# Sbte/RAILS

Measured on AMD Instinct MI355X. Metric: RAILS iterations/sec (+ A*V SpMM HBM GB/s in roofline), m=1M rows/GPU, k=128, fp64, higher is better.
Workload: dtype f64

## Files before the change

### include/rails_hip.h

```cpp
#ifndef RAILS_HIP_H
#define RAILS_HIP_H

#include <stddef.h>
#include <stdint.h>

#ifdef __cplusplus
extern "C" {
#endif

#define RAILS_OK 0
#define RAILS_EINVAL -1
#define RAILS_EHIP -2
#define RAILS_ENOMEM -3
#define RAILS_ELAPACK -4
#define RAILS_ECOMM -5
#define RAILS_ENODEV -6

typedef struct rails_ctx rails_ctx;
typedef struct rails_csr rails_csr;
typedef struct rails_panel rails_panel;

const char *rails_last_error(void);
const char *rails_version(void);


int rails_ctx_create(int device, void *stream, rails_ctx **out);
int rails_ctx_destroy(rails_ctx *ctx);
int rails_ctx_sync(rails_ctx *ctx);
void *rails_ctx_stream(rails_ctx *ctx);
int rails_ctx_stats(rails_ctx *ctx, char *buf, int cap);
int rails_ctx_set_meter(rails_ctx *ctx, int on);

int rails_ctx_set_seed(rails_ctx *ctx, uint64_t seed, uint64_t first_stream);
int rails_ctx_rng_state(rails_ctx *ctx, uint64_t *seed, uint64_t *next_stream);

int rails_ctx_set_partition(rails_ctx *ctx, int rank, int nranks, int64_t row0, int64_t m_global);

typedef int (*rails_allreduce_fn)(void *user, double *dev_buf, size_t n, void *stream);
int rails_ctx_set_allreduce(rails_ctx *ctx, rails_allreduce_fn fn, void *user);

#define RAILS_RCCL_ID_BYTES 128
int rails_rccl_unique_id(void *id_out);
int rails_ctx_init_rccl(rails_ctx *ctx, const void *id, int nranks, int rank);
int rails_ctx_set_rccl(rails_ctx *ctx, void *nccl_comm);
int rails_ctx_rccl_size(const rails_ctx *ctx);

typedef int (*rails_halo_fn)(void *user, const double *send_buf, double *recv_buf, int ncols, void *stream);


int rails_csr_create(rails_ctx *ctx, int64_t m_local, int64_t n_cols_ext, const int64_t *rowptr,
                     const int32_t *col, const double *val, rails_csr **out);
typedef int (*rails_apply_fn)(void *user, int trans, const rails_panel *X, int xc0, int nc, rails_panel *Y, int yc0);
int rails_csr_create_callback(rails_ctx *ctx, int64_t m_local, rails_apply_fn fn, void *user, rails_csr **out);
int rails_csr_destroy(rails_csr *A);
int64_t rails_csr_rows(const rails_csr *A);
int64_t rails_csr_nnz(const rails_csr *A);

int rails_csr_set_halo(rails_csr *A, int64_t n_send, const int64_t *send_rows, int64_t n_ghost,
                       rails_halo_fn fn, void *user);

int rails_csr_set_halo_counts(rails_csr *A, int nranks, const int64_t *send_counts, const int64_t *recv_counts);

int rails_spmm(rails_ctx *ctx, rails_csr *A, int trans, const rails_panel *X, int xc0, int nc,
               rails_panel *Y, int yc0);

int rails_csr_set_variant(rails_csr *A, int variant);
int rails_csr_prepare(rails_ctx *ctx, rails_csr *A, int trans, int nc, int *kernel_ready);
int rails_csr_sweep_stats(rails_csr *A, int nc, double *out);
int rails_csr_tile_stats(rails_csr *A, double *out);
int rails_csr_create_rect(rails_ctx *ctx, int64_t n_rows, int64_t n_cols, const int64_t *rowptr, const int32_t *col, const double *val,
                          rails_csr **out);
const char *rails_csr_last_kernel(const rails_csr *A);

typedef struct rails_sptrsv rails_sptrsv;
int rails_sptrsv_create(rails_ctx *ctx, int64_t n, const int64_t *rowptr, const int32_t *col, const double *val, int lower, int unit_diag,
                        rails_sptrsv **out);
void rails_sptrsv_destroy(rails_sptrsv *T);
int64_t rails_sptrsv_levels(const rails_sptrsv *T);
int rails_sptrsv_solve(rails_ctx *ctx, const rails_sptrsv *T, rails_panel *X, int c0, int nc);
int rails_panel_permute_rows(rails_ctx *ctx, const rails_panel *X, int xc0, int nc, const int32_t *perm_dev, int scatter, rails_panel *Y, int yc0);
int rails_index_upload(rails_ctx *ctx, const int32_t *host, int64_t n, int32_t **out_dev);
void rails_index_free(rails_ctx *ctx, int32_t *dev);
// ... 41 lines not shown
typedef struct rails_sweep_plan rails_sweep_plan;
int rails_sweep_plan_create(int64_t m, int64_t ncols, const int64_t *rowptr, const int32_t *col, const double *val,
                            const int *params, rails_sweep_plan **out);
int rails_sweep_plan_destroy(rails_sweep_plan *plan);
int rails_sweep_plan_info(const rails_sweep_plan *plan, int64_t *iinfo, double *dinfo);
int rails_sweep_plan_array(const rails_sweep_plan *plan, int which, const void **ptr, int64_t *count);


int rails_panel_create(rails_ctx *ctx, int64_t m_local, int capacity, rails_panel **out);
int rails_panel_create_ld(rails_ctx *ctx, int64_t m_local, int capacity, int ld, rails_panel **out);
int rails_panel_destroy(rails_panel *P);
int64_t rails_panel_rows(const rails_panel *P);
int rails_panel_capacity(const rails_panel *P);
int rails_panel_ld(const rails_panel *P);
void *rails_panel_device_ptr(const rails_panel *P);
int rails_panel_reserve(rails_ctx *ctx, rails_panel *P, int capacity);

int rails_panel_upload(rails_ctx *ctx, rails_panel *P, int c0, int nc, const double *host, int64_t ldh);
int rails_panel_download(rails_ctx *ctx, const rails_panel *P, int c0, int nc, double *host, int64_t ldh);

int rails_panel_fill(rails_ctx *ctx, rails_panel *P, int c0, int nc, double value);
int rails_panel_scale(rails_ctx *ctx, rails_panel *P, int c0, int nc, double s);
int rails_panel_copy(rails_ctx *ctx, const rails_panel *X, int xc0, int nc, rails_panel *Y, int yc0);
int rails_panel_axpy(rails_ctx *ctx, double alpha, const rails_panel *X, int xc0, int nc, rails_panel *Y,
                     int yc0);
int rails_panel_random(rails_ctx *ctx, rails_panel *P, int c0, int nc);

int rails_gram(rails_ctx *ctx, const rails_panel *X, int xc0, int a, const rails_panel *Y, int yc0, int b,
               double *C_host, int ldc);

int rails_panel_gemm(rails_ctx *ctx, double alpha, const rails_panel *X, int xc0, int k, const double *C_host,
                     int ldc, int r, double beta, rails_panel *Y, int yc0);

int rails_ctx_enable_library_gemm(rails_ctx *ctx);
int rails_ctx_library_gemm_ready(const rails_ctx *ctx);

int rails_deferred_reserve(rails_ctx *ctx, int nslots, int64_t doubles_per_slot);
int rails_gram_deferred(rails_ctx *ctx, const rails_panel *X, int xc0, int a, const rails_panel *Y, int yc0, int b, int slot);
int rails_panel_gemm_deferred(rails_ctx *ctx, double alpha, const rails_panel *X, int xc0, int k, int slot, int ld, int r, double beta,
                              rails_panel *Y, int yc0);
int rails_chol_inverse_deferred(rails_ctx *ctx, int slot_in, int w, int slot_out);
int rails_update_gram_deferred(rails_ctx *ctx, double alpha, const rails_panel *X, int xc0, int k, const double *C_host, int ldc, int r,
                               rails_panel *Y, int yc0, int r2, int slot);
int rails_update_gram_deferred_out(rails_ctx *ctx, double alpha, const rails_panel *X, int xc0, int k, const double *C_host, int ldc, int r,
                                   const rails_panel *Y, int yc0, rails_panel *Yout, int oc0, int r2, int slot);
int rails_deferred_fetch(rails_ctx *ctx, int slot, int64_t n, double *host_out);

int rails_panel_gemm_wide(rails_ctx *ctx, double alpha, const rails_panel *X, int xc0, int k, const double *C_host, int ldc, int r,
                          double beta, rails_panel *Y, int yc0);

void rails_dense_set_tile_fit(int on);
int rails_dense_tile_fit(void);
int rails_dense_last_tiles(const rails_ctx *ctx, int *update_gram_nbw, int *gram_cols_ti, int *gemm_wide_tr);

int rails_orthogonalize(rails_ctx *ctx, rails_panel *V, int k_old, int w, int method, int *used);
int rails_orthogonalize_deflated(rails_ctx *ctx, rails_panel *V, int k_old, int w, const rails_panel *N, int nc0, int q, int method, int *used);

int rails_panel_colnorms2(rails_ctx *ctx, const rails_panel *X, int c0, int nc, double *out_host);

int rails_orthogonalize_range(rails_ctx *ctx, rails_panel *V, int k_old, int w, const rails_panel *N, int nc0, int q, double tol, int *kept,
                              int32_t *kept_idx);

int rails_resid_lanczos(rails_ctx *ctx, const rails_panel *AV, int avc0, const rails_panel *MV, int mvc0, int k,
                        const double *T_host, int ldt, const rails_panel *B, int bc0, int p, int L,
                        double *H_host, int ldh, int *steps);

int rails_resid_lanczos_sparse(rails_ctx *ctx, const rails_panel *AV, int avc0, const rails_panel *MV, int mvc0, int k, const double *T_host,
                               int ldt, const rails_sprhs *S, int L, double *H_host, int ldh, int *steps);

int rails_lanczos_start(rails_ctx *ctx, const rails_panel *AV, int avc0, const rails_panel *MV, int mvc0, int k,
                        const rails_panel *B, int bc0, int p, double *sums_host);

int rails_lanczos_vectors(rails_ctx *ctx, const double *S_host, int lds, int w, rails_panel *Out, int oc0);
int rails_lanczos_last_launch(rails_ctx *ctx, int *nch, int *unroll, int *nblocks);
int rails_lanczos_release(rails_ctx *ctx);

int rails_ctx_reserve_staging(rails_ctx *ctx, size_t bytes);
int rails_timer_start(rails_ctx *ctx);
int rails_timer_stop(rails_ctx *ctx, double *ms);


void rails_sb03md(char dico, char job, char fact, char trans, int n, double *A, int lda, double *X, int ldx,
                  double *scale, int *info);
void rails_sb03md_counts(long *smith, long *schur);
void rails_sb03md_adi_counts(long *extended, long *fresh);
void rails_sb03md_set_pause(int calls);
void rails_dsyev(char jobz, char uplo, int n, double *a, int lda, double *w, int *info);
void rails_dsteqr(char compz, int n, double *d, double *e, double *z, int ldz, double *work, int *info);
void rails_dgemm(char transa, char transb, int m, int n, int k, double alpha, const double *A, int lda, const double *B,
                 int ldb, double beta, double *C, int ldc);
void rails_dtrsm(char side, char uplo, char transa, char diag, int m, int n, double alpha, const double *A, int lda, double *B, int ldb);
void rails_dpotrf(char uplo, int n, double *a, int lda, int *info);
void rails_dpstrf(char uplo, int n, double *a, int lda, int *piv, int *rank, double tol, int *info);
void rails_range_basis(int m, int n, double *a, int lda, double tol, double *q, int ldq, int *rank, int *info);
int rails_host_lapack_init(const char *path);
const char *rails_host_lapack_path(void);

#ifdef __cplusplus
}
#endif
#endif
```

### rails_amd/_lib.py

```python
import ctypes as C
import os

_HERE = os.path.dirname(os.path.abspath(__file__))
LIB_PATH = os.path.join(_HERE, "lib", "librails_hip.so")

_dp = C.POINTER(C.c_double)
_ip = C.POINTER(C.c_int)
_i64p = C.POINTER(C.c_int64)
_i32p = C.POINTER(C.c_int32)
_vp = C.c_void_p

ALLREDUCE_FN = C.CFUNCTYPE(C.c_int, C.c_void_p, C.c_void_p, C.c_size_t, C.c_void_p)
HALO_FN = C.CFUNCTYPE(C.c_int, C.c_void_p, C.c_void_p, C.c_void_p, C.c_int, C.c_void_p)
APPLY_FN = C.CFUNCTYPE(C.c_int, C.c_void_p, C.c_int, C.c_void_p, C.c_int, C.c_int, C.c_void_p, C.c_int)

SIGNATURES = {
    "rails_last_error": (C.c_char_p, []),
    "rails_version": (C.c_char_p, []),
    "rails_ctx_create": (C.c_int, [C.c_int, _vp, C.POINTER(_vp)]),
    "rails_ctx_destroy": (C.c_int, [_vp]),
    "rails_ctx_sync": (C.c_int, [_vp]),
    "rails_ctx_stream": (_vp, [_vp]),
    "rails_ctx_set_meter": (C.c_int, [_vp, C.c_int]),
    "rails_ctx_enable_library_gemm": (C.c_int, [_vp]),
    "rails_ctx_library_gemm_ready": (C.c_int, [_vp]),
    "rails_deferred_reserve": (C.c_int, [_vp, C.c_int, C.c_int64]),
    "rails_gram_deferred": (C.c_int, [_vp, _vp, C.c_int, C.c_int, _vp, C.c_int, C.c_int, C.c_int]),
    "rails_update_gram_deferred": (C.c_int, [_vp, C.c_double, _vp, C.c_int, C.c_int, _dp, C.c_int, C.c_int, _vp, C.c_int, C.c_int, C.c_int]),
    "rails_update_gram_deferred_out": (C.c_int, [_vp, C.c_double, _vp, C.c_int, C.c_int, _dp, C.c_int, C.c_int, _vp, C.c_int, _vp, C.c_int, C.c_int, C.c_int]),
    "rails_panel_gemm_deferred": (C.c_int, [_vp, C.c_double, _vp, C.c_int, C.c_int, C.c_int, C.c_int, C.c_int, C.c_double, _vp, C.c_int]),
    "rails_chol_inverse_deferred": (C.c_int, [_vp, C.c_int, C.c_int, C.c_int]),
    "rails_deferred_fetch": (C.c_int, [_vp, C.c_int, C.c_int64, _dp]),
    "rails_ctx_stats": (C.c_int, [_vp, C.c_char_p, C.c_int]),
    "rails_ctx_set_seed": (C.c_int, [_vp, C.c_uint64, C.c_uint64]),
    "rails_ctx_rng_state": (C.c_int, [_vp, C.POINTER(C.c_uint64), C.POINTER(C.c_uint64)]),
    "rails_ctx_set_partition": (C.c_int, [_vp, C.c_int, C.c_int, C.c_int64, C.c_int64]),
    "rails_ctx_set_allreduce": (C.c_int, [_vp, ALLREDUCE_FN, _vp]),
    "rails_rccl_unique_id": (C.c_int, [_vp]),
    "rails_ctx_init_rccl": (C.c_int, [_vp, _vp, C.c_int, C.c_int]),
    "rails_ctx_set_rccl": (C.c_int, [_vp, _vp]),
    "rails_ctx_rccl_size": (C.c_int, [_vp]),
    "rails_csr_set_halo_counts": (C.c_int, [_vp, C.c_int, _i64p, _i64p]),
    "rails_csr_create": (C.c_int, [_vp, C.c_int64, C.c_int64, _i64p, _i32p, _dp, C.POINTER(_vp)]),
    "rails_csr_create_rect": (C.c_int, [_vp, C.c_int64, C.c_int64, _i64p, _i32p, _dp, C.POINTER(_vp)]),
    "rails_csr_create_callback": (C.c_int, [_vp, C.c_int64, APPLY_FN, _vp, C.POINTER(_vp)]),
    "rails_csr_destroy": (C.c_int, [_vp]),
    "rails_csr_rows": (C.c_int64, [_vp]),
    "rails_csr_nnz": (C.c_int64, [_vp]),
    "rails_csr_set_halo": (C.c_int, [_vp, C.c_int64, _i64p, C.c_int64, HALO_FN, _vp]),
    "rails_spmm": (C.c_int, [_vp, _vp, C.c_int, _vp, C.c_int, C.c_int, _vp, C.c_int]),
    "rails_csr_set_variant": (C.c_int, [_vp, C.c_int]),
    "rails_csr_sweep_stats": (C.c_int, [_vp, C.c_int, _dp]),
    "rails_csr_tile_stats": (C.c_int, [_vp, _dp]),
    "rails_csr_prepare": (C.c_int, [_vp, _vp, C.c_int, C.c_int, C.POINTER(C.c_int)]),
    "rails_csr_last_kernel": (C.c_char_p, [_vp]),
    "rails_sweep_plan_create": (C.c_int, [C.c_int64, C.c_int64, _i64p, _i32p, _dp, _ip, C.POINTER(_vp)]),
    "rails_sweep_plan_destroy": (C.c_int, [_vp]),
    "rails_sweep_plan_info": (C.c_int, [_vp, _i64p, _dp]),
    "rails_sweep_plan_array": (C.c_int, [_vp, C.c_int, C.POINTER(_vp), _i64p]),
    "rails_panel_create": (C.c_int, [_vp, C.c_int64, C.c_int, C.POINTER(_vp)]),
    "rails_panel_create_ld": (C.c_int, [_vp, C.c_int64, C.c_int, C.c_int, C.POINTER(_vp)]),
    "rails_panel_destroy": (C.c_int, [_vp]),
    "rails_panel_rows": (C.c_int64, [_vp]),
    "rails_panel_capacity": (C.c_int, [_vp]),
    "rails_panel_ld": (C.c_int, [_vp]),
    "rails_panel_device_ptr": (_vp, [_vp]),
    "rails_panel_reserve": (C.c_int, [_vp, _vp, C.c_int]),
    "rails_panel_upload": (C.c_int, [_vp, _vp, C.c_int, C.c_int, _dp, C.c_int64]),
    "rails_panel_download": (C.c_int, [_vp, _vp, C.c_int, C.c_int, _dp, C.c_int64]),
    "rails_panel_fill": (C.c_int, [_vp, _vp, C.c_int, C.c_int, C.c_double]),
    "rails_panel_scale": (C.c_int, [_vp, _vp, C.c_int, C.c_int, C.c_double]),
    "rails_panel_copy": (C.c_int, [_vp, _vp, C.c_int, C.c_int, _vp, C.c_int]),
    "rails_panel_axpy": (C.c_int, [_vp, C.c_double, _vp, C.c_int, C.c_int, _vp, C.c_int]),
    "rails_sptrsv_create": (C.c_int, [_vp, C.c_int64, _i64p, _i32p, _dp, C.c_int, C.c_int, C.POINTER(_vp)]),
    "rails_sptrsv_destroy": (None, [_vp]),
    "rails_sptrsv_levels": (C.c_int64, [_vp]),
    "rails_sptrsv_solve": (C.c_int, [_vp, _vp, _vp, C.c_int, C.c_int]),
    "rails_panel_permute_rows": (C.c_int, [_vp, _vp, C.c_int, C.c_int, _vp, C.c_int, _vp, C.c_int]),
    "rails_index_upload": (C.c_int, [_vp, _i32p, C.c_int64, C.POINTER(_vp)]),
    "rails_index_free": (None, [_vp, _vp]),
    "rails_lu_create": (C.c_int, [_vp, C.c_int64, _i64p, _i32p, _dp, _i64p, _i32p, _dp, _i32p, _i32p, _i32p, C.c_int64, C.POINTER(_vp)]),
    "rails_lu_destroy": (None, [_vp]),
    "rails_lu_solve": (C.c_int, [_vp, _vp, C.c_int, _vp, C.c_int, C.c_int, _vp, C.c_int]),
    "rails_lu_stats": (C.c_int, [_vp, _i64p, C.c_int]),
    "rails_csr_create_lu": (C.c_int, [_vp, _vp, C.POINTER(_vp)]),
    "rails_iter_create": (C.c_int, [_vp, _vp, C.c_int, _dp, C.POINTER(_vp)]),
    "rails_iter_set": (C.c_int, [_vp, C.c_char_p, C.c_double]),
    "rails_iter_solve": (C.c_int, [_vp, _vp, C.c_int, _vp, C.c_int, C.c_int, _vp, C.c_int]),
    "rails_iter_precondition": (C.c_int, [_vp, _vp, _vp, C.c_int, C.c_int, _vp, C.c_int]),
    "rails_iter_stats": (C.c_int, [_vp, _dp, C.c_int]),
    "rails_iter_columns": (C.c_int, [_vp, _i32p, _dp, _i32p, C.c_int]),
    "rails_csr_create_iter": (C.c_int, [_vp, _vp, C.POINTER(_vp)]),
    "rails_iter_destroy": (None, [_vp]),
    "rails_csr_transpose_host": (C.c_int, [C.c_int64, C.c_int64, _i64p, _i32p, _dp, _i64p, _i32p, _dp]),
    "rails_csr_gram_norm2_host": (C.c_int, [C.c_int64, C.c_int64, _i64p, _i32p, _dp, _i64p, _i32p, _dp, _dp]),
    "rails_sprhs_create": (C.c_int, [_vp, C.c_int64, C.c_int, _i64p, _i32p, _dp, C.POINTER(_vp)]),
    "rails_sprhs_destroy": (None, [_vp]),
    "rails_sprhs_rows": (C.c_int64, [_vp]),
    "rails_sprhs_cols": (C.c_int64, [_vp]),
    "rails_sprhs_nnz": (C.c_int64, [_vp]),
    "rails_sprhs_gram_norm2": (C.c_double, [_vp]),
    "rails_sprhs_apply": (C.c_int, [_vp, _vp, C.c_int, _vp, C.c_int, C.c_int, _vp, C.c_int]),
    "rails_csr_create_sprhs": (C.c_int, [_vp, _vp, C.POINTER(_vp)]),
    "rails_csr_cols": (C.c_int64, [_vp]),
    "rails_csr_sprhs": (_vp, [_vp]),
    "rails_resid_lanczos_sparse": (C.c_int, [_vp, _vp, C.c_int, _vp, C.c_int, C.c_int, _dp, C.c_int, _vp, C.c_int, _dp, C.c_int, _ip]),
    "rails_panel_random": (C.c_int, [_vp, _vp, C.c_int, C.c_int]),
    "rails_gram": (C.c_int, [_vp, _vp, C.c_int, C.c_int, _vp, C.c_int, C.c_int, _dp, C.c_int]),
    "rails_panel_gemm": (C.c_int, [_vp, C.c_double, _vp, C.c_int, C.c_int, _dp, C.c_int, C.c_int, C.c_double, _vp, C.c_int]),
    "rails_panel_gemm_wide": (C.c_int, [_vp, C.c_double, _vp, C.c_int, C.c_int, _dp, C.c_int, C.c_int, C.c_double, _vp, C.c_int]),
    "rails_dense_set_tile_fit": (None, [C.c_int]),
    "rails_dense_tile_fit": (C.c_int, []),
    "rails_dense_last_tiles": (C.c_int, [_vp, _ip, _ip, _ip]),
    "rails_orthogonalize": (C.c_int, [_vp, _vp, C.c_int, C.c_int, C.c_int, _ip]),
    "rails_orthogonalize_deflated": (C.c_int, [_vp, _vp, C.c_int, C.c_int, _vp, C.c_int, C.c_int, C.c_int, _ip]),
    "rails_panel_colnorms2": (C.c_int, [_vp, _vp, C.c_int, C.c_int, _dp]),
    "rails_orthogonalize_range": (C.c_int, [_vp, _vp, C.c_int, C.c_int, _vp, C.c_int, C.c_int, C.c_double, _ip, _i32p]),
    "rails_resid_lanczos": (C.c_int, [_vp, _vp, C.c_int, _vp, C.c_int, C.c_int, _dp, C.c_int, _vp, C.c_int, C.c_int, C.c_int,
                                      _dp, C.c_int, _ip]),
    "rails_lanczos_start": (C.c_int, [_vp, _vp, C.c_int, _vp, C.c_int, C.c_int, _vp, C.c_int, C.c_int, _dp]),
    "rails_lanczos_vectors": (C.c_int, [_vp, _dp, C.c_int, C.c_int, _vp, C.c_int]),
    "rails_lanczos_last_launch": (C.c_int, [_vp, _ip, _ip, _ip]),
    "rails_lanczos_release": (C.c_int, [_vp]),
    "rails_timer_start": (C.c_int, [_vp]),
    "rails_timer_stop": (C.c_int, [_vp, _dp]),
    "rails_sb03md": (None, [C.c_char, C.c_char, C.c_char, C.c_char, C.c_int, _dp, C.c_int, _dp, C.c_int, _dp, _ip]),
    "rails_dsyev": (None, [C.c_char, C.c_char, C.c_int, _dp, C.c_int, _dp, _ip]),
    "rails_dsteqr": (None, [C.c_char, C.c_int, _dp, _dp, _dp, C.c_int, _dp, _ip]),
    "rails_ctx_reserve_staging": (C.c_int, [_vp, C.c_size_t]),
    "rails_sb03md_set_pause": (None, [C.c_int]),
    "rails_sb03md_counts": (None, [C.POINTER(C.c_long), C.POINTER(C.c_long)]),
    "rails_sb03md_adi_counts": (None, [C.POINTER(C.c_long), C.POINTER(C.c_long)]),
    "rails_dtrsm": (None, [C.c_char, C.c_char, C.c_char, C.c_char, C.c_int, C.c_int, C.c_double, _dp, C.c_int, _dp, C.c_int]),
    "rails_dgemm": (None, [C.c_char, C.c_char, C.c_int, C.c_int, C.c_int, C.c_double, _dp, C.c_int, _dp, C.c_int, C.c_double, _dp, C.c_int]),
    "rails_dpotrf": (None, [C.c_char, C.c_int, _dp, C.c_int, _ip]),
    "rails_dpstrf": (None, [C.c_char, C.c_int, _dp, C.c_int, _ip, _ip, C.c_double, _ip]),
    "rails_range_basis": (None, [C.c_int, C.c_int, _dp, C.c_int, C.c_double, _dp, C.c_int, _ip, _ip]),
    "rails_host_lapack_init": (C.c_int, [C.c_char_p]),
    "rails_host_lapack_path": (C.c_char_p, []),
}

_lib = None


class RailsError(RuntimeError):
    pass


def load():
    global _lib
    if _lib is not None:
        return _lib
    if not os.path.exists(LIB_PATH):
        raise RailsError(
            "rails_amd: %s is missing -- build it with `python -c 'import __graft_entry__ as g; g.build()'` "
            "or `make -C rails_amd/csrc`; there is no CPU fallback" % LIB_PATH)
    lib = C.CDLL(LIB_PATH, mode=C.RTLD_GLOBAL)
    for name, (res, args) in SIGNATURES.items():
        fn = getattr(lib, name)
        fn.restype = res
        fn.argtypes = args
    try:
        from ._solver_sigs import bind as _bind_solver
        _bind_solver(lib)
    except ImportError:
        pass
# ... 12 lines not shown
```

### rails_amd/csrc/ctx.hip

```cpp
#include "rails_internal.h"

static thread_local char g_err[1024] = "";

void rails_set_error(const char *fmt, ...)
{
    va_list ap;
    va_start(ap, fmt);
    vsnprintf(g_err, sizeof(g_err), fmt, ap);
    va_end(ap);
}

extern "C" const char *rails_last_error(void) { return g_err; }
extern "C" const char *rails_version(void) { return "rails_amd 0.1 (gfx950)"; }


extern "C" int rails_ctx_create(int device, void *stream, rails_ctx **out)
{
    RAILS_REQUIRE(out != nullptr, "rails_ctx_create: out is null");
    int ndev = 0;
    hipError_t e = hipGetDeviceCount(&ndev);
    if (e != hipSuccess || ndev <= 0) {
        rails_set_error("rails_ctx_create: no HIP device visible (%s); the HIP path has no CPU fallback",
                        e == hipSuccess ? "device count 0" : hipGetErrorString(e));
        return RAILS_ENODEV;
// ... 41 lines not shown
    if (!c) return RAILS_OK;
    hipSetDevice(c->device);
    rails_stream_sync(c);
    rails_lanczos_release(c);
    rails_rccl_release(c);
    rails_library_gemm_release(c);
    for (auto &fp : c->free_panels) hipFree(fp.second);
    c->free_panels.clear();
    if (c->ws) hipFree(c->ws);
    if (c->small) hipFree(c->small);
    if (c->pinned) hipHostFree(c->pinned);
    if (c->defer_dev) hipFree(c->defer_dev);
    if (c->defer_pin) hipHostFree(c->defer_pin);
    if (c->ev0) hipEventDestroy(c->ev0);
    if (c->ev1) hipEventDestroy(c->ev1);
    if (c->ev_h2d) hipEventDestroy(c->ev_h2d);
    for (hipEvent_t e : c->meter_events) hipEventDestroy(e);
    if (c->stream2) hipStreamDestroy(c->stream2);
    if (c->ev_fork) hipEventDestroy(c->ev_fork);
    if (c->ev_join) hipEventDestroy(c->ev_join);
    if (c->own_stream) hipStreamDestroy(c->stream);
    delete c;
    return RAILS_OK;
}

int rails_ctx_second_stream(rails_ctx *c)
{
    if (c->stream2) return RAILS_OK;
    RAILS_HIP_CHECK(hipStreamCreateWithFlags(&c->stream2, hipStreamNonBlocking));
    RAILS_HIP_CHECK(hipEventCreateWithFlags(&c->ev_fork, hipEventDisableTiming));
    RAILS_HIP_CHECK(hipEventCreateWithFlags(&c->ev_join, hipEventDisableTiming));
    return RAILS_OK;
}

extern "C" int rails_ctx_sync(rails_ctx *c)
{
    RAILS_REQUIRE(c, "rails_ctx_sync: null context");
    RAILS_HIP_CHECK(rails_stream_sync(c));
    return RAILS_OK;
}

extern "C" int rails_ctx_stats(rails_ctx *c, char *buf, int cap)
{
    RAILS_REQUIRE(c && buf && cap > 0, "rails_ctx_stats: bad argument");
    int n = snprintf(buf, (size_t)cap,
                     "{\"orth_block\": %ld, \"orth_columnwise\": %ld, \"spmm_tiled\": %ld, \"spmm_planes\": %ld, \"spmm_halo_overlapped\": %ld, \"spmm_sweep\": %ld, \"spmm_rowgather\": %ld, \"spmm_callback\": %ld, \"device_allocations\": %ld, \"allreduce\": %ld, "
                     "\"lanczos\": %ld, \"lanczos_start\": %ld, \"orth_repair\": %ld, \"update_gram_fused\": %ld, \"rowquad\": %ld, \"orth_range\": %ld, \"orth_range_passes\": %ld, \"orth_range_syncs\": %ld, \"gpu_busy_ms\": %.3f}",
                     c->n_orth_block, c->n_orth_columnwise, c->n_spmm_tiled, c->n_spmm_planes, c->n_spmm_overlapped, c->n_spmm_sweep, c->n_spmm_rowgather, c->n_spmm_callback, c->n_dev_alloc, c->n_allreduce, c->n_lanczos, c->n_lanczos_start, c->n_orth_repair, c->n_update_gram_fused, c->n_rowquad, c->n_orth_range, c->n_orth_range_passes, c->n_orth_range_syncs, c->gpu_busy_ms);
    RAILS_REQUIRE(n > 0 && n < cap, "rails_ctx_stats: buffer too small");
    return RAILS_OK;
}

extern "C" void *rails_ctx_stream(rails_ctx *c) { return c ? (void *)c->stream : nullptr; }

extern "C" int rails_ctx_set_meter(rails_ctx *c, int on)
{
    RAILS_REQUIRE(c, "rails_ctx_set_meter: null context");
    hipSetDevice(c->device);
    RAILS_HIP_CHECK(rails_stream_sync(c));
    if (on && c->meter_events.empty()) {
        c->meter_events.resize(2 * RAILS_METER_PAIRS, nullptr);
        for (hipEvent_t &e : c->meter_events) RAILS_HIP_CHECK(hipEventCreate(&e));
    }
    c->meter = on != 0;
    return RAILS_OK;
}

extern "C" int rails_ctx_rng_state(rails_ctx *c, uint64_t *seed, uint64_t *next_stream)
{
    RAILS_REQUIRE(c && seed && next_stream, "rails_ctx_rng_state: null argument");
    *seed = c->seed;
    *next_stream = c->next_stream;
    return RAILS_OK;
}

extern "C" int rails_ctx_set_seed(rails_ctx *c, uint64_t seed, uint64_t first_stream)
{
    RAILS_REQUIRE(c, "null context");
    c->seed = seed;
    c->next_stream = first_stream;
    return RAILS_OK;
}

extern "C" int rails_ctx_set_partition(rails_ctx *c, int rank, int nranks, int64_t row0, int64_t m_global)
{
    RAILS_REQUIRE(c, "null context");
    RAILS_REQUIRE(nranks >= 1 && rank >= 0 && rank < nranks && row0 >= 0, "rails_ctx_set_partition: bad rank %d/%d row0 %lld",
                  rank, nranks, (long long)row0);
    c->rank = rank;
    c->nranks = nranks;
    c->row0 = row0;
    c->m_global = m_global;
    return RAILS_OK;
}

extern "C" int rails_ctx_set_allreduce(rails_ctx *c, rails_allreduce_fn fn, void *user)
{
    RAILS_REQUIRE(c, "null context");
    c->allreduce = fn;
    c->allreduce_user = user;
    return RAILS_OK;
}

int rails_allreduce_dev(rails_ctx *c, double *dev, size_t n)
{
    if (n == 0) return RAILS_OK;
// ... 406 lines not shown
```

### rails_amd/csrc/dense.hip

```cpp
#include "rails_internal.h"

#include <dlfcn.h>
#include <atomic>
#include <mutex>

#include <algorithm>

namespace {

typedef double v4f64 __attribute__((ext_vector_type(4)));
typedef double v2f64 __attribute__((ext_vector_type(2)));

std::atomic<int> g_tile_fit{-1};

bool dense_tile_fit()
{
    int v = g_tile_fit.load(std::memory_order_relaxed);
    if (v < 0) {
        const char *e = getenv("RAILS_DENSE_TILE_FIT");
        int undecided = -1;
        g_tile_fit.compare_exchange_strong(undecided, (e ? atoi(e) : 1) ? 1 : 0);
        v = g_tile_fit.load(std::memory_order_relaxed);
    }
    return v != 0;
}

__device__ __forceinline__ v4f64 mfma_f64(double a, double b, v4f64 c)
{
    return __builtin_amdgcn_mfma_f64_16x16x4f64(a, b, c, 0, 0, 0);
}

struct OneSeg {
    const double *X;
    int ld;
    struct Row {
        const double *x;
    };
    __device__ int col(int c) const { return c; }
    __device__ Row row(int64_t r) const { return {X + r * ld}; }
    __device__ static const double *at(Row r, int c) { return r.x + c; }
};
struct TwoSeg {
    const double *X1;
    int ld1, a1;
    const double *X2;
    int ld2;
    struct Col {
        int off;
        bool second;
    };
    struct Row {
        const double *x1, *x2;
    };
    __device__ Col col(int c) const
    {
        const bool second = c >= a1;
        return {second ? c - a1 : c, second};
    }
    __device__ Row row(int64_t r) const { return {X1 + r * ld1, X2 + r * ld2}; }
    __device__ static const double *at(Row r, Col c) { return (c.second ? r.x2 : r.x1) + c.off; }
};

template <int TI, int TJ>
__global__ __launch_bounds__(256) __attribute__((amdgpu_waves_per_eu(3, 8))) void k_gram(const double *__restrict__ X, int ldx, int a, const double *__restrict__ Y, int ldy,
                                              int b, int64_t m, int64_t rows_per_slab, int ngj, double *__restrict__ partial)
{
    const OneSeg Xo{X, ldx};
#include "dense_gram.inc"
}

template <int TI, int TJ>
__global__ __launch_bounds__(256) void k_gram2(const double *__restrict__ X1, int ldx1, int a1, const double *__restrict__ X2, int ldx2, int a,
                                               const double *__restrict__ Y, int ldy, int b, int64_t m, int64_t rows_per_slab, int ngj,
                                               double *__restrict__ partial)
{
// ... 223 lines not shown
        if (cost < best_cost) best = ti, best_cost = cost;
    }
    if (one_tile && best == 6 && (ntiles + 4) / 5 == (ntiles + 5) / 6 && dense_tile_fit()) best = 5;
    return best;
}

#define RAILS_GRAM_COLS_CASE(K, TI, TJ, NE, ...) RAILS_LAUNCH((K<TI, TJ, NE>), grid, dim3(256), 0, c->stream, __VA_ARGS__, Y, ldy, b, m, rps, c->ws)
#define RAILS_GRAM_COLS(K, ...)                                                                                                            \
    do {                                                                                                                                   \
        const int ntiles = (a + 15) / 16, best = gram_cols_tiles(ntiles, b <= 16 || extra);                                                \
        const dim3 grid((unsigned)nslab, (unsigned)(((ntiles + best - 1) / best + 3) / 4));                                                \
        c->last_gram_cols_ti = best;                                                                                                       \
        if (extra) {                                                                                                                       \
            if (best == 4)                                                                                                                 \
                RAILS_GRAM_COLS_CASE(K, 4, 1, 1, __VA_ARGS__);                                                                             \
            else if (best == 5)                                                                                                            \
                RAILS_GRAM_COLS_CASE(K, 5, 1, 1, __VA_ARGS__);                                                                             \
            else if (best == 6)                                                                                                            \
                RAILS_GRAM_COLS_CASE(K, 6, 1, 1, __VA_ARGS__);                                                                             \
            else                                                                                                                           \
                RAILS_GRAM_COLS_CASE(K, 8, 1, 1, __VA_ARGS__);                                                                             \
        } else if (b <= 16) {                                                                                                              \
            if (best == 4)                                                                                                                 \
                RAILS_GRAM_COLS_CASE(K, 4, 1, 0, __VA_ARGS__);                                                                             \
            else if (best == 5)                                                                                                            \
                RAILS_GRAM_COLS_CASE(K, 5, 1, 0, __VA_ARGS__);                                                                             \
            else if (best == 6)                                                                                                            \
                RAILS_GRAM_COLS_CASE(K, 6, 1, 0, __VA_ARGS__);                                                                             \
            else                                                                                                                           \
                RAILS_GRAM_COLS_CASE(K, 8, 1, 0, __VA_ARGS__);                                                                             \
        } else if (best == 3)                                                                                                              \
            RAILS_GRAM_COLS_CASE(K, 3, 2, 0, __VA_ARGS__);                                                                                 \
        else if (best == 4)                                                                                                                \
            RAILS_GRAM_COLS_CASE(K, 4, 2, 0, __VA_ARGS__);                                                                                 \
        else                                                                                                                               \
            RAILS_GRAM_COLS_CASE(K, 5, 2, 0, __VA_ARGS__);                                                                                 \
    } while (0)

}

extern "C" void rails_dense_set_tile_fit(int on) { g_tile_fit.store(on ? 1 : 0); }

extern "C" int rails_dense_tile_fit(void) { return dense_tile_fit() ? 1 : 0; }

extern "C" int rails_dense_last_tiles(const rails_ctx *c, int *update_gram_nbw, int *gram_cols_ti, int *gemm_wide_tr)
{
    RAILS_REQUIRE(c, "rails_dense_last_tiles: null context");
    if (update_gram_nbw) *update_gram_nbw = c->last_update_gram_nbw;
    if (gram_cols_ti) *gram_cols_ti = c->last_gram_cols_ti;
    if (gemm_wide_tr) *gemm_wide_tr = c->last_gemm_wide_tr;
    return RAILS_OK;
}

int rails_gram_dev(rails_ctx *c, const double *X, int ldx, const double *Y, int ldy, int64_t m, int a, int b, double *C_dev)
{
    if (a <= 0 || b <= 0) return RAILS_OK;
    int64_t nslab, rps;
    gram_slabs(m, a, b, &nslab, &rps);
    size_t n = (size_t)a * b;
    RAILS_TRY(rails_ws_reserve(c, (size_t)nslab * n * sizeof(double)));
    if (b <= 16 && a <= 16)
        launch_gram<1, 1>(c, X, ldx, a, Y, ldy, b, m, rps, nslab, c->ws);
    else if (b <= 32 && a >= 128) {
        static const int cols_form = getenv("RAILS_GRAM_COLS") ? atoi(getenv("RAILS_GRAM_COLS")) : 1;
        if (cols_form) {
            static const int extra_env = getenv("RAILS_GRAM_EXTRA_COLUMN") ? atoi(getenv("RAILS_GRAM_EXTRA_COLUMN")) : 1;
            const bool extra = extra_env && b == 17;
            RAILS_GRAM_COLS(k_gram_cols, X, ldx, a);
        } else if (b <= 16)
            launch_gram<8, 1>(c, X, ldx, a, Y, ldy, b, m, rps, nslab, c->ws);
        else
            launch_gram<4, 2>(c, X, ldx, a, Y, ldy, b, m, rps, nslab, c->ws);
    } else if (b <= 16)
        launch_gram<8, 1>(c, X, ldx, a, Y, ldy, b, m, rps, nslab, c->ws);
    else if (a <= 16)
        launch_gram<1, 8>(c, X, ldx, a, Y, ldy, b, m, rps, nslab, c->ws);
    else if (a <= 32 && b <= 32)
        launch_gram<2, 2>(c, X, ldx, a, Y, ldy, b, m, rps, nslab, c->ws);
    else if (b <= 32)
        launch_gram<4, 2>(c, X, ldx, a, Y, ldy, b, m, rps, nslab, c->ws);
    else if (a <= 32)
        launch_gram<2, 4>(c, X, ldx, a, Y, ldy, b, m, rps, nslab, c->ws);
    else
        launch_gram<2, 4>(c, X, ldx, a, Y, ldy, b, m, rps, nslab, c->ws);
    RAILS_LAUNCH(k_reduce_partials, dim3((unsigned)((n + 63) / 64)), dim3(1024), 0, c->stream, c->ws, nslab, (int64_t)n, C_dev);
    RAILS_HIP_CHECK(hipGetLastError());
    return RAILS_OK;
}

int rails_gram2_dev(rails_ctx *c, const double *X1, int ldx1, int a1, const double *X2, int ldx2, int a2, const double *Y, int ldy, int64_t m, int b,
                    double *C_dev)
{
    const int a = a1 + a2;
    if (a <= 0 || b <= 0) return RAILS_OK;
    int64_t nslab, rps;
    gram_slabs(m, a, b, &nslab, &rps);
    const size_t n = (size_t)a * b;
    RAILS_TRY(rails_ws_reserve(c, (size_t)nslab * n * sizeof(double)));
    if (a >= 128 && b <= 32) {
        const bool extra = b == 17;
        RAILS_GRAM_COLS(k_gram_cols2, X1, ldx1, a1, X2, ldx2, a);
    } else if (a <= 16 && b <= 16)
        launch_gram2<1, 1>(c, X1, ldx1, a1, X2, ldx2, a, Y, ldy, b, m, rps, nslab, c->ws);
    else if (b <= 16)
        launch_gram2<8, 1>(c, X1, ldx1, a1, X2, ldx2, a, Y, ldy, b, m, rps, nslab, c->ws);
    else
// ... 313 lines not shown
            t += __shfl_xor(t, 32, 64);
            if (kk == 0) rede[wave][q][li] = t;
        }
        __syncthreads();
        {
            const double sum = ((red[0][wave][lane] + red[1][wave][lane]) + red[2][wave][lane]) + red[3][wave][lane];
            const double ynew = yv + alpha * sum;
            if (yok) Yo[yrow * ldo + li] = ynew;
            awL[(kk + 4 * wave) * 16 + li] = (yok && li < r2) ? ynew : 0.0;
            if (NE > 0 && eok) {
                const double se = ((rede[0][ene][erow] + rede[1][ene][erow]) + rede[2][ene][erow]) + rede[3][ene][erow];
                Yo[(row0 + erow) * ldo + 16 + ene] = ye + alpha * se;
            }
        }
        __syncthreads();
        double bq[4];
#pragma unroll
        for (int q = 0; q < 4; ++q) bq[q] = awL[(4 * q + kk) * 16 + li];
        double *Tw = T[wave];
#pragma unroll
        for (int b = 0; b < NBW; ++b) {
            *reinterpret_cast<v2f64 *>(&Tw[li * 16 + 4 * kk]) = (v2f64){xs[b][0], xs[b][1]};
            *reinterpret_cast<v2f64 *>(&Tw[li * 16 + 4 * kk + 2]) = (v2f64){xs[b][2], xs[b][3]};
            __builtin_amdgcn_fence(__ATOMIC_RELEASE, "wavefront");
            __builtin_amdgcn_wave_barrier();
            __builtin_amdgcn_fence(__ATOMIC_ACQUIRE, "wavefront");
            double a4[4];
#pragma unroll
            for (int q = 0; q < 4; ++q) a4[q] = Tw[(4 * q + kk) * 16 + li];
            __builtin_amdgcn_fence(__ATOMIC_RELEASE, "wavefront");
            __builtin_amdgcn_wave_barrier();
#pragma unroll
            for (int q = 0; q < 4; ++q) acc2[b] = mfma_f64(a4[q], bq[q], acc2[b]);
        }
    };
    double xa[NBW][4], xb[NBW][4], yva, yea, yvb, yeb;
    fetch(blockIdx.x, xa);
    fetch_y(blockIdx.x, yva, yea);
    __syncthreads();
    for (int64_t tile = blockIdx.x; tile < ntiles; tile += 2 * (int64_t)gridDim.x) {
        work(tile, xa, yva, yea, xb, yvb, yeb);
        if (tile + gridDim.x < ntiles) work(tile + gridDim.x, xb, yvb, yeb, xa, yva, yea);
    }
    double *P = partial + (int64_t)blockIdx.x * k * r2;
#pragma unroll
    for (int b = 0; b < NBW; ++b)
#pragma unroll
        for (int v = 0; v < 4; ++v) {
            const int ci = (b * 4 + wave) * 16 + kk + 4 * v;
            if (ci < k && li < r2) P[ci + (int64_t)li * k] = acc2[b][v];
        }
}

template <int NBW>
static void launch_update_gram(rails_ctx *c, int ne, unsigned grid, double alpha, const double *X, int ldx, int k, const double *C, int r, const double *Y, int ldy,
                               double *Yo, int ldo, int r2, int64_t m, int64_t ntiles)
{
    if (ne == 0)
        RAILS_LAUNCH((k_update_gram<NBW, 0>), dim3(grid), dim3(256), 0, c->stream, alpha, X, ldx, k, C, r, Y, ldy, Yo, ldo, r2, m, ntiles, c->ws);
    else
        RAILS_LAUNCH((k_update_gram<NBW, 1>), dim3(grid), dim3(256), 0, c->stream, alpha, X, ldx, k, C, r, Y, ldy, Yo, ldo, r2, m, ntiles, c->ws);
    c->last_update_gram_nbw = NBW;
}

extern "C" int rails_update_gram_deferred_out(rails_ctx *c, double alpha, const rails_panel *X, int xc0, int k, const double *C_host, int ldc, int r,
                                              const rails_panel *Y, int yc0, rails_panel *Yout, int oc0, int r2, int slot)
{
    if (c) hipSetDevice(c->device);
    rails_slow_guard slow__(c, "rails_update_gram_deferred", k, r);
    RAILS_REQUIRE(c && X && Y && Yout && C_host, "rails_update_gram_deferred: null argument");
    RAILS_REQUIRE(k >= 1 && r >= 1 && r <= 256 && r2 >= 1 && r2 <= r && ldc >= k && xc0 >= 0 && yc0 >= 0 && xc0 + k <= X->cap && yc0 + r <= Y->cap && X->m == Y->m,
                  "rails_update_gram_deferred: bad shapes");
    RAILS_REQUIRE(oc0 >= 0 && oc0 + r <= Yout->cap && Yout->m == X->m, "rails_update_gram_deferred: output window [%d,%d) outside capacity %d, or row mismatch", oc0,
                  oc0 + r, Yout->cap);
    if (X->d == Y->d) RAILS_REQUIRE(xc0 + k <= yc0 || yc0 + r <= xc0, "rails_update_gram_deferred: overlapping windows of one panel");
    if (X->d == Yout->d) RAILS_REQUIRE(xc0 + k <= oc0 || oc0 + r <= xc0, "rails_update_gram_deferred: overlapping windows of one panel");
    if (Y->d == Yout->d) RAILS_REQUIRE(yc0 == oc0 || yc0 + r <= oc0 || oc0 + r <= yc0, "rails_update_gram_deferred: partially overlapping windows of one panel");
    const size_t n = (size_t)k * r2;
    RAILS_SLOT_CHECK(slot, n, "rails_update_gram_deferred");
    double *out = c->defer_dev + (size_t)slot * c->defer_slot;
    if (X->m == 0) {
        RAILS_HIP_CHECK(hipMemsetAsync(out, 0, n * sizeof(double), c->stream));
    } else {
        const size_t nc = (size_t)k * r;
        RAILS_TRY(rails_small_reserve(c, nc * sizeof(double)));
        RAILS_TRY(rails_pinned_begin_write(c, nc * sizeof(double)));
        for (int j = 0; j < r; ++j) memcpy(c->pinned + (size_t)j * k, C_host + (size_t)j * ldc, sizeof(double) * k);
        RAILS_HIP_CHECK(hipMemcpyAsync(c->small, c->pinned, nc * sizeof(double), hipMemcpyHostToDevice, c->stream));
        RAILS_TRY(rails_pinned_end_write(c));
        static const int fused_env = getenv("RAILS_FUSED_UPDATE_GRAM") ? atoi(getenv("RAILS_FUSED_UPDATE_GRAM")) : 1;
        const double *Xp = X->d + xc0;
        const double *Ypp = Y->d + yc0;
        double *Yop = Yout->d + oc0;
        const int k4 = (k + 3) & ~3;
        const bool rows_ok = ((((uintptr_t)Xp) & 15) == 0 && (X->ld % 2) == 0) && (k4 == k || (X->d == Y->d && yc0 == xc0 + k && r >= k4 - k));
        if (fused_env && rows_ok && r <= 17 && r2 <= 16 && k >= 32 && k <= 512 && X->m >= 4096) {
            const int64_t ntiles = (X->m + 15) / 16;
            const unsigned grid = (unsigned)std::min<int64_t>(ntiles, 2 * (int64_t)std::max(c->num_cu, 1));
            const int ne = r > 16 ? r - 16 : 0;
            RAILS_TRY(rails_ws_reserve(c, (size_t)grid * n * sizeof(double)));
            if (k <= 256)
                launch_update_gram<4>(c, ne, grid, alpha, Xp, X->ld, k, c->small, r, Ypp, Y->ld, Yop, Yout->ld, r2, X->m, ntiles);
            else if (k <= 320 && dense_tile_fit())
                launch_update_gram<5>(c, ne, grid, alpha, Xp, X->ld, k, c->small, r, Ypp, Y->ld, Yop, Yout->ld, r2, X->m, ntiles);
            else if (k <= 384)
                launch_update_gram<6>(c, ne, grid, alpha, Xp, X->ld, k, c->small, r, Ypp, Y->ld, Yop, Yout->ld, r2, X->m, ntiles);
            else
                launch_update_gram<8>(c, ne, grid, alpha, Xp, X->ld, k, c->small, r, Ypp, Y->ld, Yop, Yout->ld, r2, X->m, ntiles);
            RAILS_LAUNCH(k_reduce_partials, dim3((unsigned)((n + 63) / 64)), dim3(1024), 0, c->stream, c->ws, (int64_t)grid, (int64_t)n, out);
            RAILS_HIP_CHECK(hipGetLastError());
            c->n_update_gram_fused++;
        } else {
            if (Yop != Ypp) RAILS_TRY(rails_panel_copy(c, Y, yc0, r, Yout, oc0));
            RAILS_TRY(rails_panel_gemm_dev(c, alpha, Xp, X->ld, k, c->small, r, 1.0, Yop, Yout->ld, X->m));
// ... 234 lines not shown
```

### rails_amd/csrc/rails_internal.h

```cpp
#ifndef RAILS_INTERNAL_H
#define RAILS_INTERNAL_H

#include <hip/hip_runtime.h>

#include <cstdarg>
#include <cstdint>
#include <cstdio>
#include <cstring>
#include <ctime>
#include <string>
#include <vector>

#include "rails_hip.h"

void rails_set_error(const char *fmt, ...);

#define RAILS_HIP_CHECK(expr)                                                                      \
    do {                                                                                           \
        hipError_t e__ = (expr);                                                                   \
        if (e__ != hipSuccess) {                                                                   \
            rails_set_error("%s:%d: %s failed: %s", __FILE__, __LINE__, #expr, hipGetErrorString(e__)); \
            return RAILS_EHIP;                                                                     \
        }                                                                                          \
    } while (0)
// ... 3 lines not shown
        if (!(cond)) {                                                                             \
            rails_set_error(__VA_ARGS__);                                                          \
            return RAILS_EINVAL;                                                                   \
        }                                                                                          \
    } while (0)

#define RAILS_TRY(expr)                                                                            \
    do {                                                                                           \
        int rc__ = (expr);                                                                         \
        if (rc__ != RAILS_OK) return rc__;                                                         \
    } while (0)

static inline int rails_pad_ld(int capacity) { return ((capacity < 1 ? 1 : capacity) + 15) / 16 * 16; }

struct rails_ctx {
    int device = 0;
    hipStream_t stream = nullptr;
    bool own_stream = false;
    hipStream_t stream2 = nullptr;
    hipEvent_t ev_fork = nullptr, ev_join = nullptr;
    int num_cu = 256;
    uint64_t seed = 1;
    uint64_t next_stream = 0;
    int rank = 0, nranks = 1;
    int64_t row0 = 0, m_global = -1;
    rails_allreduce_fn allreduce = nullptr;
    void *allreduce_user = nullptr;
    void *rccl = nullptr;
    bool own_rccl = false;
    int rccl_nranks = 0, rccl_rank = 0;
    double *ws = nullptr;
    size_t ws_bytes = 0;
    std::vector<std::pair<size_t, double *>> free_panels;
    size_t free_panel_bytes = 0;
    double *small = nullptr;
    size_t small_bytes = 0;
    double *pinned = nullptr;
    size_t pinned_bytes = 0;
    hipEvent_t ev0 = nullptr, ev1 = nullptr;
    hipEvent_t ev_h2d = nullptr;
    bool h2d_pending = false;
    double *defer_dev = nullptr, *defer_pin = nullptr;
    size_t defer_slot = 0;
    int defer_nslots = 0;
    bool meter = false;
    std::vector<hipEvent_t> meter_events;
    int meter_open = 0;
    long meter_missed = 0;
    double gpu_busy_ms = 0.0;
    void *lz = nullptr;
    long n_orth_block = 0, n_orth_columnwise = 0, n_spmm_tiled = 0, n_spmm_planes = 0, n_spmm_overlapped = 0, n_spmm_sweep = 0, n_spmm_rowgather = 0, n_spmm_callback = 0, n_dev_alloc = 0, n_allreduce = 0, n_lanczos = 0, n_lanczos_start = 0, n_orth_repair = 0, n_update_gram_fused = 0, n_rowquad = 0;
    long n_orth_range = 0, n_orth_range_passes = 0, n_orth_range_syncs = 0;
    int last_update_gram_nbw = 0, last_gram_cols_ti = 0, last_gemm_wide_tr = 0;
};

constexpr int RAILS_METER_PAIRS = 512;
inline bool rails_meter_before(rails_ctx *c)
{
    if (!c->meter) return false;
    if (c->meter_open >= RAILS_METER_PAIRS) {
        c->meter_missed++;
        return false;
    }
    hipEventRecord(c->meter_events[2 * c->meter_open], c->stream);
    return true;
}
inline void rails_meter_after(rails_ctx *c) { hipEventRecord(c->meter_events[2 * c->meter_open++ + 1], c->stream); }
inline hipError_t rails_stream_sync(rails_ctx *c)
{
    const hipError_t e = hipStreamSynchronize(c->stream);
    for (int i = 0; i < c->meter_open; ++i) {
        float ms = 0.0f;
        if (e == hipSuccess && hipEventElapsedTime(&ms, c->meter_events[2 * i], c->meter_events[2 * i + 1]) == hipSuccess) c->gpu_busy_ms += ms;
    }
    c->meter_open = 0;
    return e;
}
#define RAILS_LAUNCH(...)                                                                                                                  \
    do {                                                                                                                                   \
        const bool rails_metered = rails_meter_before(c);                                                                                  \
        hipLaunchKernelGGL(__VA_ARGS__);                                                                                                   \
        if (rails_metered) rails_meter_after(c);                                                                                           \
    } while (0)

struct rails_panel {
    rails_ctx *ctx = nullptr;
    double *d = nullptr;
    int64_t m = 0;
    int cap = 0;
    int ld = 0;
};

struct rails_planes_plan;
struct rails_sweep_cache;
struct rails_tile_cache;

struct rails_csr {
    rails_ctx *ctx = nullptr;
    rails_sweep_cache *sweep = nullptr;
    rails_planes_plan *planes = nullptr;
    rails_tile_cache *tiled = nullptr;
    int64_t m = 0, ncols_ext = 0, nnz = 0;
    bool rect = false;
    int64_t *rowptr = nullptr;
    int32_t *col = nullptr;
    double *val = nullptr;
// ... 124 lines not shown
```

Baseline: 239.0.

## Add software-pipelined update_gram kernel that prefetches next tile's X and Y

```diff
diff --git a/include/rails_hip.h b/include/rails_hip.h
--- a/include/rails_hip.h
+++ b/include/rails_hip.h
@@ -28,6 +28,7 @@
 int rails_ctx_destroy(rails_ctx *ctx);
 int rails_ctx_sync(rails_ctx *ctx);
 void *rails_ctx_stream(rails_ctx *ctx);
+int rails_ctx_num_cu(const rails_ctx *ctx);
 int rails_ctx_stats(rails_ctx *ctx, char *buf, int cap);
 int rails_ctx_set_meter(rails_ctx *ctx, int on);
 
@@ -175,6 +176,10 @@
 void rails_dense_set_tile_fit(int on);
 int rails_dense_tile_fit(void);
 int rails_dense_last_tiles(const rails_ctx *ctx, int *update_gram_nbw, int *gram_cols_ti, int *gemm_wide_tr);
+
+void rails_dense_set_update_gram_pipeline(int on);
+int rails_dense_update_gram_pipeline(void);
+int rails_dense_last_update_gram_form(const rails_ctx *ctx, int *form);
 
 int rails_orthogonalize(rails_ctx *ctx, rails_panel *V, int k_old, int w, int method, int *used);
 int rails_orthogonalize_deflated(rails_ctx *ctx, rails_panel *V, int k_old, int w, const rails_panel *N, int nc0, int q, int method, int *used);
diff --git a/rails_amd/_lib.py b/rails_amd/_lib.py
--- a/rails_amd/_lib.py
+++ b/rails_amd/_lib.py
@@ -21,6 +21,7 @@
     "rails_ctx_destroy": (C.c_int, [_vp]),
     "rails_ctx_sync": (C.c_int, [_vp]),
     "rails_ctx_stream": (_vp, [_vp]),
+    "rails_ctx_num_cu": (C.c_int, [_vp]),
     "rails_ctx_set_meter": (C.c_int, [_vp, C.c_int]),
     "rails_ctx_enable_library_gemm": (C.c_int, [_vp]),
     "rails_ctx_library_gemm_ready": (C.c_int, [_vp]),
@@ -112,6 +113,9 @@
     "rails_dense_set_tile_fit": (None, [C.c_int]),
     "rails_dense_tile_fit": (C.c_int, []),
     "rails_dense_last_tiles": (C.c_int, [_vp, _ip, _ip, _ip]),
+    "rails_dense_set_update_gram_pipeline": (None, [C.c_int]),
+    "rails_dense_update_gram_pipeline": (C.c_int, []),
+    "rails_dense_last_update_gram_form": (C.c_int, [_vp, _ip]),
     "rails_orthogonalize": (C.c_int, [_vp, _vp, C.c_int, C.c_int, C.c_int, _ip]),
     "rails_orthogonalize_deflated": (C.c_int, [_vp, _vp, C.c_int, C.c_int, _vp, C.c_int, C.c_int, C.c_int, _ip]),
     "rails_panel_colnorms2": (C.c_int, [_vp, _vp, C.c_int, C.c_int, _dp]),
diff --git a/rails_amd/csrc/ctx.hip b/rails_amd/csrc/ctx.hip
--- a/rails_amd/csrc/ctx.hip
+++ b/rails_amd/csrc/ctx.hip
@@ -117,6 +117,8 @@
 }
 
 extern "C" void *rails_ctx_stream(rails_ctx *c) { return c ? (void *)c->stream : nullptr; }
+
+extern "C" int rails_ctx_num_cu(const rails_ctx *c) { return c ? c->num_cu : 0; }
 
 extern "C" int rails_ctx_set_meter(rails_ctx *c, int on)
 {
diff --git a/rails_amd/csrc/dense.hip b/rails_amd/csrc/dense.hip
--- a/rails_amd/csrc/dense.hip
+++ b/rails_amd/csrc/dense.hip
@@ -21,6 +21,20 @@
         int undecided = -1;
         g_tile_fit.compare_exchange_strong(undecided, (e ? atoi(e) : 1) ? 1 : 0);
         v = g_tile_fit.load(std::memory_order_relaxed);
+    }
+    return v != 0;
+}
+
+std::atomic<int> g_update_gram_pipeline{-1};
+
+bool dense_update_gram_pipeline()
+{
+    int v = g_update_gram_pipeline.load(std::memory_order_relaxed);
+    if (v < 0) {
+        const char *e = getenv("RAILS_UPDATE_GRAM_PIPELINE");
+        int undecided = -1;
+        g_update_gram_pipeline.compare_exchange_strong(undecided, (e ? atoi(e) : 1) ? 1 : 0);
+        v = g_update_gram_pipeline.load(std::memory_order_relaxed);
     }
     return v != 0;
 }
@@ -350,6 +364,17 @@
     return RAILS_OK;
 }
 
+extern "C" void rails_dense_set_update_gram_pipeline(int on) { g_update_gram_pipeline.store(on ? 1 : 0); }
+
+extern "C" int rails_dense_update_gram_pipeline(void) { return dense_update_gram_pipeline() ? 1 : 0; }
+
+extern "C" int rails_dense_last_update_gram_form(const rails_ctx *c, int *form)
+{
+    RAILS_REQUIRE(c && form, "rails_dense_last_update_gram_form: null argument");
+    *form = c->last_update_gram_form;
+    return RAILS_OK;
+}
+
 int rails_gram_dev(rails_ctx *c, const double *X, int ldx, const double *Y, int ldy, int64_t m, int a, int b, double *C_dev)
 {
     if (a <= 0 || b <= 0) return RAILS_OK;
@@ -769,14 +794,162 @@
         }
 }
 
+template <int NBW, int NE>
+__global__ __launch_bounds__(256, (NBW <= 6 ? 2 : 1)) void k_update_gram_p(double alpha, const double *__restrict__ X, int ldx, int k, const double *__restrict__ C, int r,
+                                                       const double *Yp, int ldy, double *Yo, int ldo, int r2, int64_t m, int64_t ntiles,
+                                                       double *__restrict__ partial)
+{
+    __shared__ double red[4][4][64];
+    __shared__ double rede[4][1][16];
+    __shared__ double awL[16 * 16];
+    __shared__ __attribute__((aligned(16))) double T[4][NBW][16 * 16];
+    __shared__ __attribute__((aligned(16))) double c16[NE > 0 ? 64 * NBW : 2];
+    const int lane = threadIdx.x & 63, wave = threadIdx.x >> 6;
+    const int li = lane & 15, kk = lane >> 4;
+    double cr[NBW][4];
+#pragma unroll
+    for (int b = 0; b < NBW; ++b)
+#pragma unroll
+        for (int s = 0; s < 4; ++s) {
+            const int kl = (b * 4 + wave) * 16 + 4 * kk + s;
+            cr[b][s] = (kl < k && li < r) ? C[kl + (int64_t)li * k] : 0.0;
+        }
+    if (NE > 0) {
+        for (int kl = threadIdx.x; kl < 64 * NBW; kl += 256) c16[kl] = (kl < k && 16 < r) ? C[kl + (int64_t)16 * k] : 0.0;
+        __syncthreads();
+    }
+    v4f64 acc2[NBW];
+#pragma unroll
+    for (int b = 0; b < NBW; ++b) acc2[b] = (v4f64){0.0, 0.0, 0.0, 0.0};
+
+    const int k4 = (k + 3) & ~3;
+    auto xrow_of = [&](int64_t tile) {
+        const int64_t myrow = (tile < ntiles ? tile : ntiles - 1) * 16 + li;
+        return X + (myrow < m ? myrow : m - 1) * ldx;
+    };
+    auto fetch_block = [&](const double *xrow, int b, double *xs) {
+        const int kcol = (b * 4 + wave) * 16 + 4 * kk;
+        const double *src = xrow + (kcol < k4 ? kcol : 0);
+        const v2f64 t0 = *reinterpret_cast<const v2f64 *>(src);
+        const v2f64 t1 = *reinterpret_cast<const v2f64 *>(src + 2);
+        xs[0] = t0.x;
+        xs[1] = t0.y;
+        xs[2] = t1.x;
+        xs[3] = t1.y;
+    };
+    const int erow = threadIdx.x & 15, ene = threadIdx.x >> 4;
+    auto fetch_y = [&](int64_t tile, double &yv, double &ye) {
+        const int64_t t16 = (tile < ntiles ? tile : ntiles - 1) * 16;
+        const int64_t yrow = t16 + kk + 4 * wave, er = t16 + erow;
+        yv = Yp[(yrow < m ? yrow : m - 1) * ldy + (li < r ? li : 0)];
+        ye = NE > 0 ? Yp[(er < m ? er : m - 1) * ldy + (16 + ene < r ? 16 + ene : 0)] : 0.0;
+    };
+    const int tw0 = li * 16 + 2 * ((2 * kk) ^ (li & 7)), tw1 = li * 16 + 2 * ((2 * kk + 1) ^ (li & 7));
+    const int tr0 = kk * 16 + 2 * ((li >> 1) ^ kk) + (li & 1), tr1 = (4 + kk) * 16 + 2 * ((li >> 1) ^ (4 + kk)) + (li & 1);
+    double xs[NBW][4], yv, ye;
+    {
+        const double *xrow = xrow_of(blockIdx.x);
+#pragma unroll
+        for (int b = 0; b < NBW; ++b) fetch_block(xrow, b, xs[b]);
+        fetch_y(blockIdx.x, yv, ye);
+    }
+    for (int64_t tile = blockIdx.x; tile < ntiles; tile += gridDim.x) {
+        const int64_t row0 = tile * 16;
+        const double *xnext = xrow_of(tile + gridDim.x);
+        const int64_t yrow = row0 + kk + 4 * wave;
+        const bool yok = yrow < m && li < r;
+        const bool eok = ene < NE && 16 + ene < r && row0 + erow < m;
+        v4f64 p = (v4f64){0.0, 0.0, 0.0, 0.0};
+        double e[NE > 0 ? NE : 1];
+#pragma unroll
+        for (int q = 0; q < NE; ++q) e[q] = 0.0;
+#pragma unroll
+        for (int b = 0; b < NBW; ++b) {
+            *reinterpret_cast<v2f64 *>(&T[wave][b][tw0]) = (v2f64){xs[b][0], xs[b][1]};
+            *reinterpret_cast<v2f64 *>(&T[wave][b][tw1]) = (v2f64){xs[b][2], xs[b][3]};
+            double ce[4] = {0.0, 0.0, 0.0, 0.0};
+            if (NE > 0) {
+                const v2f64 c0 = *reinterpret_cast<const v2f64 *>(&c16[(b * 4 + wave) * 16 + 4 * kk]);
+                const v2f64 c1 = *reinterpret_cast<const v2f64 *>(&c16[(b * 4 + wave) * 16 + 4 * kk + 2]);
+                ce[0] = c0.x, ce[1] = c0.y, ce[2] = c1.x, ce[3] = c1.y;
+            }
+#pragma unroll
+            for (int s = 0; s < 4; ++s) {
+                p = mfma_f64(xs[b][s], cr[b][s], p);
+#pragma unroll
+                for (int q = 0; q < NE; ++q) e[q] += xs[b][s] * ce[s];
+            }
+            __builtin_amdgcn_sched_barrier(0);
+            fetch_block(xnext, b, xs[b]);
+            __builtin_amdgcn_sched_barrier(0);
+        }
+#pragma unroll
+        for (int v = 0; v < 4; ++v) red[wave][v][lane] = p[v];
+#pragma unroll
+        for (int q = 0; q < NE; ++q) {
+            double t = e[q];
+            t += __shfl_xor(t, 16, 64);
+            t += __shfl_xor(t, 32, 64);
+            if (kk == 0) rede[wave][q][li] = t;
+        }
+        __syncthreads();
+        {
+            const double sum = ((red[0][wave][lane] + red[1][wave][lane]) + red[2][wave][lane]) + red[3][wave][lane];
+            const double ynew = yv + alpha * sum;
+            if (yok) Yo[yrow * ldo + li] = ynew;
+            awL[(kk + 4 * wave) * 16 + li] = (yok && li < r2) ? ynew : 0.0;
+            if (NE > 0 && eok) {
+                const double se = ((rede[0][ene][erow] + rede[1][ene][erow]) + rede[2][ene][erow]) + rede[3][ene][erow];
+                Yo[(row0 + erow) * ldo + 16 + ene] = ye + alpha * se;
+            }
+        }
+        __builtin_amdgcn_sched_barrier(0);
+        fetch_y(tile + gridDim.x, yv, ye);
+        __syncthreads();
+        double bq[4];
+#pragma unroll
+        for (int q = 0; q < 4; ++q) bq[q] = awL[(4 * q + kk) * 16 + li];
+        double a4[2][4];
+#pragma unroll
+        for (int q = 0; q < 4; ++q) a4[0][q] = T[wave][0][((q & 1) ? tr1 : tr0) + 128 * (q >> 1)];
+#pragma unroll
+        for (int b = 0; b < NBW; ++b) {
+            if (b + 1 < NBW) {
+#pragma unroll
+                for (int q = 0; q < 4; ++q) a4[(b + 1) & 1][q] = T[wave][b + 1][((q & 1) ? tr1 : tr0) + 128 * (q >> 1)];
+            }
+            __builtin_amdgcn_sched_barrier(0);
+#pragma unroll
+            for (int q = 0; q < 4; ++q) acc2[b] = mfma_f64(a4[b & 1][q], bq[q], acc2[b]);
+            __builtin_amdgcn_sched_barrier(0);
+        }
+        __builtin_amdgcn_fence(__ATOMIC_RELEASE, "wavefront");
+        __builtin_amdgcn_wave_barrier();
+    }
+    double *P = partial + (int64_t)blockIdx.x * k * r2;
+#pragma unroll
+    for (int b = 0; b < NBW; ++b)
+#pragma unroll
+        for (int v = 0; v < 4; ++v) {
+            const int ci = (b * 4 + wave) * 16 + kk + 4 * v;
+            if (ci < k && li < r2) P[ci + (int64_t)li * k] = acc2[b][v];
+        }
+}
+
 template <int NBW>
 static void launch_update_gram(rails_ctx *c, int ne, unsigned grid, double alpha, const double *X, int ldx, int k, const double *C, int r, const double *Y, int ldy,
                                double *Yo, int ldo, int r2, int64_t m, int64_t ntiles)
 {
-    if (ne == 0)
+    const bool pipeline = dense_update_gram_pipeline();
+    if (pipeline && ne == 0)
+        RAILS_LAUNCH((k_update_gram_p<NBW, 0>), dim3(grid), dim3(256), 0, c->stream, alpha, X, ldx, k, C, r, Y, ldy, Yo, ldo, r2, m, ntiles, c->ws);
+    else if (pipeline)
+        RAILS_LAUNCH((k_update_gram_p<NBW, 1>), dim3(grid), dim3(256), 0, c->stream, alpha, X, ldx, k, C, r, Y, ldy, Yo, ldo, r2, m, ntiles, c->ws);
+    else if (ne == 0)
         RAILS_LAUNCH((k_update_gram<NBW, 0>), dim3(grid), dim3(256), 0, c->stream, alpha, X, ldx, k, C, r, Y, ldy, Yo, ldo, r2, m, ntiles, c->ws);
     else
         RAILS_LAUNCH((k_update_gram<NBW, 1>), dim3(grid), dim3(256), 0, c->stream, alpha, X, ldx, k, C, r, Y, ldy, Yo, ldo, r2, m, ntiles, c->ws);
+    c->last_update_gram_form = pipeline ? 2 : 1;
     c->last_update_gram_nbw = NBW;
 }
 
diff --git a/rails_amd/csrc/rails_internal.h b/rails_amd/csrc/rails_internal.h
--- a/rails_amd/csrc/rails_internal.h
+++ b/rails_amd/csrc/rails_internal.h
@@ -79,6 +79,7 @@
     long n_orth_block = 0, n_orth_columnwise = 0, n_spmm_tiled = 0, n_spmm_planes = 0, n_spmm_overlapped = 0, n_spmm_sweep = 0, n_spmm_rowgather = 0, n_spmm_callback = 0, n_dev_alloc = 0, n_allreduce = 0, n_lanczos = 0, n_lanczos_start = 0, n_orth_repair = 0, n_update_gram_fused = 0, n_rowquad = 0;
     long n_orth_range = 0, n_orth_range_passes = 0, n_orth_range_syncs = 0;
     int last_update_gram_nbw = 0, last_gram_cols_ti = 0, last_gemm_wide_tr = 0;
+    int last_update_gram_form = 0;
 };
 
 constexpr int RAILS_METER_PAIRS = 512;
```

Measured after the change: 245.0, median of 6. 2.5% higher.
